# bootphon/abnet3

Hardware: AMD Instinct MI355X
Metric: frame-pairs/sec (Siamese train step: fwd both towers + coscos2 + bwd + Adadelta) (higher is better)
Workload: dtype f16x2; 1 GPU; C2: SiameseNetwork 40->500x2->100 sigmoid, coscos2(avg=False), Adadelta(0.1), 4096 frame pairs per GPU per step, 40-d N(0,1) frames; pairs_per_gpu=4096, global_pairs=4096, parallelism=dp1, graph_replay=False, dp_gradient_buckets=1

## Files before the change

### abnet3_amd/csrc/common.h

```cpp
#pragma once
#include <hip/hip_runtime.h>
#include <stdint.h>
#include <stdio.h>

#include "../../include/abnet3_hip.h"

namespace abn {

void set_error(const char* fmt, ...);

#define ABN_REQUIRE(cond, ...)                      \
    do {                                            \
        if (!(cond)) {                              \
            ::abn::set_error(__VA_ARGS__);          \
            return ABN_E_ARG;                       \
        }                                           \
    } while (0)

#define ABN_CHECK_LAUNCH(what)                                               \
    do {                                                                     \
        hipError_t e_ = hipGetLastError();                                   \
        if (e_ != hipSuccess) {                                              \
            ::abn::set_error("%s: %s", what, hipGetErrorString(e_));         \
            return ABN_E_LAUNCH;                                             \
        }                                                                    \
    } while (0)

struct Switches {
    bool planes;
    bool fused;
    int64_t fused_min_rows;
    bool bn_planes;
    bool bn_persist;
    bool wgrad_xcd;
    bool bf16x3_planes;
    bool bwd_pair;
    int gemm_tile;
    bool dtw_f40, dtw_pc;
    int wgrad_tile128;
    int dtw_wgs_per_cu;
    int wgrad_wgs_heavy, wgrad_wgs_light;
    int64_t wgrad_rows_per_slab;
    bool wide;
    int64_t wide_max_rows;
    int wide_max_groups;
    bool wgrad_step;
    bool dtw_dealt;
    int oneshot_wgs;
    int knn_split;
};
const Switches& switches();
void reload_switches();

// ... 23 lines not shown
```

### abnet3_amd/csrc/tower.hip

```cpp
#include <stdarg.h>
#include <stdlib.h>
#include <string.h>

#include <math.h>
#include <atomic>

#include "common.h"
#include "gemm_f32.h"
#include "opt_rule.h"
#include "tower_fused.h"
#include "tower_planes.h"
#include "tower_bn_persist.h"
#include "tower_wide.h"
#include "tower_wgrad_step.h"

namespace abn {

static thread_local char g_err[512] = "";
void set_error(const char* fmt, ...)
{
    va_list ap;
    va_start(ap, fmt);
    vsnprintf(g_err, sizeof(g_err), fmt, ap);
    va_end(ap);
// ... 10 lines not shown
    s.bn_persist = !off("ABN_BN_PERSIST");
    s.wgrad_xcd = !off("ABN_WGRAD_XCD");
    s.bf16x3_planes = !off("ABN_BF16X3_PLANES");
    s.bwd_pair = !off("ABN_BWD_PAIR");
    s.gemm_tile = getenv("ABN_GEMM_TILE") ? atoi(getenv("ABN_GEMM_TILE")) : -1;
    s.wgrad_rows_per_slab = getenv("ABN_WGRAD_ROWS_PER_SLAB") ? atoll(getenv("ABN_WGRAD_ROWS_PER_SLAB")) : -1;
    s.wide = !off("ABN_WIDE");
    s.wide_max_rows = getenv("ABN_WIDE_MAX_ROWS") ? atoll(getenv("ABN_WIDE_MAX_ROWS")) : -1;
    s.wide_max_groups = getenv("ABN_WIDE_MAXG") ? atoi(getenv("ABN_WIDE_MAXG")) : WD_MAXG;
    if (s.wide_max_groups < 1 || s.wide_max_groups > WD_MAXG) s.wide_max_groups = WD_MAXG;
    s.dtw_f40 = !off("ABN_DTW_F40");
    s.dtw_pc = !off("ABN_DTW_PC");
    s.wgrad_wgs_heavy = getenv("ABN_WGRAD_WGS_HEAVY") ? atoi(getenv("ABN_WGRAD_WGS_HEAVY")) : 128;
    s.wgrad_wgs_light = getenv("ABN_WGRAD_WGS_LIGHT") ? atoi(getenv("ABN_WGRAD_WGS_LIGHT")) : 128;
    s.wgrad_tile128 = getenv("ABN_WGRAD_TILE128") ? atoi(getenv("ABN_WGRAD_TILE128")) : -1;
    s.dtw_wgs_per_cu = getenv("ABN_DTW_WGS") ? atoi(getenv("ABN_DTW_WGS")) : 6;
    if (s.dtw_wgs_per_cu < 1 || s.dtw_wgs_per_cu > 9) s.dtw_wgs_per_cu = 6;
    s.wgrad_step = !off("ABN_WGRAD_STEP");
    s.dtw_dealt = !off("ABN_DTW_SCHED");
    s.oneshot_wgs = getenv("ABN_ONESHOT_WGS") ? atoi(getenv("ABN_ONESHOT_WGS")) : 32;
    if (s.oneshot_wgs < 1 || s.oneshot_wgs > 256) s.oneshot_wgs = 32;
    s.knn_split = getenv("ABN_KNN_SPLIT") ? atoi(getenv("ABN_KNN_SPLIT")) : 0;
    if (s.knn_split < 0) s.knn_split = 0;
    return s;
}
static Switches g_switches = read_switches();
const Switches& switches() { return g_switches; }
void reload_switches() { g_switches = read_switches(); }

template <int BM, int BN, bool A_KC, bool B_KC, int EPI, bool VEC, int BF16>
// ... 751 lines not shown
{
    bool all3 = np == 2 && w.n_layers > 0;
    for (int i = 0; i < w.n_layers; ++i) all3 = all3 && w.L[i].shape == 3;
    return all3;
}
constexpr size_t WGRAD128_LDS = (size_t)4 * 8 * 2048 + 128;
static void launch_wgrad(int np, const WgradP& w, int n_wg, hipStream_t st)
{
#ifndef WG128_GENERAL
    if (wgrad_all128(np, w)) {
        static bool attr_set[16] = {};
        int dev = 0;
        (void)hipGetDevice(&dev);
        dev = (dev >= 0 && dev < 16) ? dev : 0;
        if (!attr_set[dev]) {
            (void)hipFuncSetAttribute(reinterpret_cast<const void*>(wgrad_planes128_kernel), hipFuncAttributeMaxDynamicSharedMemorySize, (int)WGRAD128_LDS);
            attr_set[dev] = true;
        }
        hipLaunchKernelGGL(wgrad_planes128_kernel, dim3((unsigned)n_wg), dim3(PL_NT), WGRAD128_LDS, st, w);
        return;
    }
#endif
    PL_LAUNCH(np, wgrad_planes_kernel, dim3((unsigned)n_wg), dim3(PL_NT), wgrad_all128(np, w) ? WGRAD128_LDS : wgrad_lds_of(np), st, w);
}
static inline int gemm_prec(int precision) { return precision > 2 ? 2 : precision; }
static inline bool bn_sync_on(const abn_tower_desc* t) { return t->bn_sync_fn != nullptr && t->bn_sync_world >= 1; }
static inline int64_t bn_wgs_per_call(int64_t rows, int64_t n_calls) { return (rows / n_calls + PL_ROWS - 1) / PL_ROWS; }
static inline int64_t bn_vrows(int64_t rows, int64_t n_calls) { return n_calls * bn_wgs_per_call(rows, n_calls) * PL_ROWS; }
static bool planes_dims_ok(const abn_tower_desc* t)
{
    if (t->precision < 1) return false;
    for (int l = 0; l <= t->n_layers; ++l)
        if (t->dims[l] < 4 || t->dims[l] > PL_MAXW || t->dims[l] % 4 != 0) return false;
    return true;
// ... 176 lines not shown
    const int64_t n = in_dim + 1;
    const int64_t tm128 = (out_dim + 127) / 128, tm64 = (out_dim + 63) / 64;
    const int64_t tn128 = (n + 127) / 128, tn64 = (n + 63) / 64;
    const int64_t est = out_dim > 64 ? tm128 * tn64 : (n > 64 ? tm64 * tn128 : tm64 * tn64);
    int64_t s = (512 + est - 1) / est;
    const int64_t by_rows = rows / 128 < 1 ? 1 : rows / 128;
    if (s > by_rows) s = by_rows;
    if (s > MAX_SPLITS) s = MAX_SPLITS;
    return (int)(s < 1 ? 1 : s);
}

static inline bool wgrad_tile128(int64_t rows, bool np2)
{
    const int mode = switches().wgrad_tile128;
    return np2 && mode != 0 && (mode > 0 || (rows + 63) / 64 * 64 >= 2048);
}
static int planes_split_count(int64_t rows, int64_t out_dim, int64_t in_dim, bool np2 = false)
{
    int shape, bn, bk;
    const int nblk = pl_blocks(out_dim), kblk = pl_blocks(in_dim + 1);
    wgrad_shape(nblk, kblk, &shape, &bn, &bk, wgrad_tile128(rows, np2));
    const int64_t tiles = (int64_t)((nblk + bn - 1) / bn) * ((kblk + bk - 1) / bk);
    int64_t s = (128 + tiles - 1) / tiles;
    if (shape == 3) { const int64_t want = tiles >= 16 ? switches().wgrad_wgs_heavy : switches().wgrad_wgs_light; s = (want + tiles - 1) / tiles; }
    const int64_t r64 = (rows + 63) / 64 * 64;
    const int64_t per = switches().wgrad_rows_per_slab > 0 ? switches().wgrad_rows_per_slab : 128;
    const int64_t by_rows = r64 / per < 1 ? 1 : r64 / per;
    const int64_t cap = shape == 0 ? MAX_SPLITS : 2 * MAX_SPLITS;
    if (s > by_rows) s = by_rows;
    if (s > cap) s = cap;
// ... 335 lines not shown
    }
    b.a_top = ws + L.a[nl - 1];
    b.dx = dx;
    b.drop_seed = reinterpret_cast<const unsigned long long*>(t->drop_seed);
    b.drop_p = t->drop_p;
    const PackLayout PL = make_pack_layout(t);
    const char* const image = t->wpack ? reinterpret_cast<const char*>(t->wpack) : reinterpret_cast<const char*>(ws + L.wpack);
    for (int l = 0; l <= nl; ++l) b.dims[l] = (int)t->dims[l];
    for (int l = 0; l < nl; ++l) {
        b.act[l] = (l == nl - 1) ? t->last_act : t->act;
        b.tp[l] = reinterpret_cast<const char*>(ws + L.tp[l]);
        b.mask[l] = t->drop_mask[l];
        b.wpt[l] = image + PL.wpt[l];
        b.dzp[l] = reinterpret_cast<char*>(scratch + B.dzp[l]);
        b.amax_dz[l] = B.amax_dz[l] >= 0 ? scratch + B.amax_dz[l] : nullptr;
    }
    b.wbase = image; b.wbytes = PL.bytes;
    int l_first, l_end;
    { const int rc = wgrad_range(t, &l_first, &l_end); if (rc != ABN_OK) return rc; }
    if (t->wgrad_part == 2) part = PLANES_BWD_WGRAD;
    int n_wg = 0;
    const WgradP w = make_wgrad(t, rows, L, B, ws, scratch, &n_wg, l_first, l_end);
    static bool bw_attr_set[16] = {};
    int dev = 0;
    (void)hipGetDevice(&dev);
    dev = (dev >= 0 && dev < 16) ? dev : 0;
    if (!bw_attr_set[dev]) {
        PL_LDS_ATTR(tower_dgrad_planes_kernel, pl_lds_bytes);
        PL_LDS_ATTR(wgrad_planes_kernel, wgrad_lds_of);
        bw_attr_set[dev] = true;
    }
    const dim3 cgrid((unsigned)((rows + PL_ROWS - 1) / PL_ROWS));
    const bool do_dgrad = part != PLANES_BWD_WGRAD, do_wgrad = part != PLANES_BWD_DGRAD;
    if (do_dgrad) PL_LAUNCH(np, tower_dgrad_planes_kernel, cgrid, dim3(PL_NT), pl_lds_bytes(np), st, b);
    if (do_wgrad && n_wg > 0) launch_wgrad(np, w, n_wg, st);
    ABN_CHECK_LAUNCH("tower_backward (planes)");
    if (t->defer_reduce) return ABN_OK;
// ... 420 lines not shown
        const void* kernels[3][3] = {
            {reinterpret_cast<const void*>(tower_fwd_planes_kernel<1, PL_TRAIN>), reinterpret_cast<const void*>(tower_fwd_planes_kernel<1, PL_INFER>),
             reinterpret_cast<const void*>(tower_fwd_planes_kernel<1, PL_INFER_BN>)},
            {reinterpret_cast<const void*>(tower_fwd_planes_kernel<2, PL_TRAIN>), reinterpret_cast<const void*>(tower_fwd_planes_kernel<2, PL_INFER>),
             reinterpret_cast<const void*>(tower_fwd_planes_kernel<2, PL_INFER_BN>)},
            {reinterpret_cast<const void*>(tower_fwd_planes_kernel<3, PL_TRAIN>), reinterpret_cast<const void*>(tower_fwd_planes_kernel<3, PL_INFER>),
             reinterpret_cast<const void*>(tower_fwd_planes_kernel<3, PL_INFER_BN>)}};
        if (!pl_attr_set[dev]) {
            for (int a = 0; a < 3; ++a)
                for (int m = 0; m < 3; ++m)
                    if (kernels[a][m])
                        (void)hipFuncSetAttribute(kernels[a][m], hipFuncAttributeMaxDynamicSharedMemorySize,
                                                  (int)(m == PL_INFER_BN ? pl_lds_bytes_bn(a + 1) : pl_lds_bytes_stag(a + 1)));
            pl_attr_set[dev] = true;
        }
        void* kargs[] = {&f};
        (void)hipLaunchKernel(kernels[np - 1][mode], fgrid, dim3(PL_NT), kargs, lds, st);
        ABN_CHECK_LAUNCH("tower_fwd_planes");
        return ABN_OK;
    }
    if (fusable) {
        FusedFwdP f = {};
        f.n_layers = t->n_layers;
        f.rows = (int)rows;
        f.rows_call = (int)rpc;
        f.bf16 = gemm_prec(t->precision);
        f.x1 = x1; f.x2 = x2;
        f.x_copy = x2 ? ws + L.x : nullptr;
        for (int l = 0; l <= t->n_layers; ++l) f.dims[l] = (int)t->dims[l];
        for (int l = 0; l < t->n_layers; ++l) {
// ... 497 lines not shown
```

### abnet3_amd/csrc/tower_planes.h

```cpp
#pragma once
#include <type_traits>

#include "gemm_f32.h"

namespace abn {

typedef int v4i __attribute__((ext_vector_type(4)));

constexpr int PL_ROWS = 32;
constexpr int PL_WAVES = 8;
constexpr int PL_NT = 64 * PL_WAVES;
constexpr int PL_MAXW = 512;
constexpr int PL_MAXSTEPS = PL_MAXW / 16;
#ifdef PL_DEPTH_OVERRIDE
constexpr int PL_DEPTH = PL_DEPTH_OVERRIDE;
#else
constexpr int PL_DEPTH = 4;
#endif
constexpr int PL_PART_BYTES = 4 * 16 * 64 * 4;
constexpr int PL_SC_BYTES = PL_WAVES * 64 * 4 + PL_WAVES * 32 * 4;
constexpr int PL_AMAX = 32;

__host__ __device__ inline int pl_steps(int64_t contraction) { return ((int)((contraction + 15) / 16) + PL_DEPTH - 1) / PL_DEPTH * PL_DEPTH; }
__host__ __device__ inline int pl_blocks(int64_t features) { return (int)((features + 31) / 32); }
// ... 128 lines not shown
    for (int s = 0; s < 2; ++s) {
        if constexpr (NP == 2) {
            f16x8 o;
#pragma unroll
            for (int j = 0; j < 8; ++j) o[j] = (_Float16)((16 * s + 8 * (j >> 2) + 4 * h + (j & 3)) == c ? 1.0f : 0.0f);
            idf[s] = __builtin_bit_cast(bf16x8, o);
        } else {
#pragma unroll
            for (int j = 0; j < 8; ++j) idf[s][j] = (__bf16)((16 * s + 8 * (j >> 2) + 4 * h + (j & 3)) == c ? 1.0f : 0.0f);
        }
    }
}

template <int NP>
__device__ __forceinline__ void emit_planes(char* dst, const Frag<NP> f[2], const bf16x8 idf[2], int lane, int ones_c, int rows_left,
                                            const float* __restrict__ inv_tab = nullptr)
{
    const int c = lane & 31, h = lane >> 5;
    f32x16 t;
#pragma unroll
    for (int pl = 0; pl < NP; ++pl) {
        f32x16 u;
#pragma unroll
        for (int q = 0; q < 16; ++q) u[q] = 0.0f;
        u = pl_mfma<NP>(f[0].p[pl], idf[0], u);
        u = pl_mfma<NP>(f[1].p[pl], idf[1], u);
        if (pl == 0) t = u;
        else t += u;
    }
    if constexpr (NP == 2) {
#pragma unroll
        for (int g = 0; g < 4; ++g) {
            const f32x4 iv = *reinterpret_cast<const f32x4*>(inv_tab + 8 * g + 4 * h);
#pragma unroll
            for (int e = 0; e < 4; ++e) t[4 * g + e] *= iv[e];
        }
    }
    if (c == ones_c) {
#pragma unroll
        for (int q = 0; q < 16; ++q) t[q] = (q & 3) + 8 * (q >> 2) + 4 * h < rows_left ? 1.0f : 0.0f;
    }
#pragma unroll
    for (int s = 0; s < 2; ++s) {
        if constexpr (NP >= 2) {
            char* o = dst + s * 2048 + lane * 16;
            *reinterpret_cast<f32x4*>(o) = f32x4{t[8 * s], t[8 * s + 1], t[8 * s + 2], t[8 * s + 3]};
            *reinterpret_cast<f32x4*>(o + 1024) = f32x4{t[8 * s + 4], t[8 * s + 5], t[8 * s + 6], t[8 * s + 7]};
        } else {
            bf16x8 o;
#pragma unroll
            for (int j = 0; j < 8; ++j) o[j] = (__bf16)t[8 * s + j];
            *reinterpret_cast<bf16x8*>(dst + s * 1024 + lane * 16) = o;
        }
    }
}

template <int NP>
__device__ __forceinline__ int tgather_row_offset(int r)
{
    const int sp = r >> 4, jh = (r >> 3) & 1, jl = r & 3, hp = (r >> 2) & 1;
    if constexpr (NP >= 2) return sp * 2048 + jh * 1024 + hp * 32 * 16 + jl * 4;
    else return sp * 1024 + hp * 32 * 16 + (4 * jh + jl) * 2;
}
template <int NP>
__device__ __forceinline__ float tgather(const char* tile_pair, int row_off, int c)
{
    if constexpr (NP >= 2) return *reinterpret_cast<const float*>(tile_pair + row_off + c * 16);
    else return (float)*reinterpret_cast<const __bf16*>(tile_pair + row_off + c * 16);
}

template <int N> __device__ __forceinline__ void wait_vmcnt() { asm volatile("s_waitcnt vmcnt(%0)" :: "n"(N) : "memory"); }

struct PackJob {
    const float* W;
    int N, K;
    int transposed;
    int nblk, nsteps;
    int tile0;
    int blk0;
    int64_t dst;
};
struct PackTable {
    int n_jobs, n_tiles, n_blocks;
// ... 267 lines not shown
    int rows_call;
    int dims[ABN_MAX_LAYERS + 1];
    int act[ABN_MAX_LAYERS];
    const float* x1;
    const float* x2;
    float* x_copy;
    const char* wp[ABN_MAX_LAYERS];
    const char* wbase;
    int64_t wbytes;
    const float* b[ABN_MAX_LAYERS];
    const float* mask[ABN_MAX_LAYERS];
    float* out[ABN_MAX_LAYERS];
    char* tp[ABN_MAX_LAYERS];
    int64_t tp_steps;
    float* amax[ABN_MAX_LAYERS];
    const unsigned long long* drop_seed;
    float drop_p;
    const float* bn_rm[ABN_MAX_LAYERS];
    const float* bn_rv[ABN_MAX_LAYERS];
    const float* bn_w[ABN_MAX_LAYERS];
    const float* bn_b[ABN_MAX_LAYERS];
    float bn_eps;
    float* bn_part;
#ifdef ABN_STAMPS
    unsigned long long* stamps;
#endif
};

enum { PL_TRAIN = 0, PL_INFER = 1, PL_INFER_BN = 2, PL_BN_TRAIN = 3 };

// ... 334 lines not shown
        if (rescale) park_max();
    } else if (ws.active && ws.khalf == 1) {
#pragma unroll
        for (int q = 0; q < 16; ++q) part[((wave & 3) * 16 + q) * 64 + lane] = acc[0][q];
    }
    PSTAMPF(4 + 5 * l);
    __syncthreads();
    PSTAMPF(5 + 5 * l);
    if constexpr (STAGC) { if (stag_on) st.in_halves = false; }
    if (KS == 2 && ws.active && ws.khalf == 0) {
#pragma unroll
        for (int q = 0; q < 16; ++q) acc[0][q] += part[(wave * 16 + q) * 64 + lane];
        finish();
    }
    float osc = 1.0f;
    if (rescale) {
        if (KS == 2) { park_max(); __syncthreads(); }
        float oinv;
        const float m = row_scales(sc, wave, lane, osc, oinv);
        ainv = oinv;
        if (!INFER && p.tp[l + 1] && wave == 0) store_amax_rows(p.amax[l + 1] + (int64_t)blockIdx.x * PL_AMAX, m, 1.0f, lane);
    }
    const float* const inv_tab = sc + PL_WAVES * 64 + wave * 32;
    float* __restrict__ out = p.out[l];
    char* const tp = !INFER && !BNT && l + 1 < p.n_layers ? p.tp[l + 1] : nullptr;
    if (BNT && ws.active && ws.khalf == 0) {
        float* const pw = p.bn_part + (int64_t)blockIdx.x * (3 * PL_MAXW);
#pragma unroll
        for (int j = 0; j < BPW; ++j) {
            if (blk0 + j >= nblk) continue;
#pragma unroll
            for (int g = 0; g < 4; ++g) {
                f32x4 sd, sq, cc;
#pragma unroll
                for (int e = 0; e < 4; ++e) {
                    const float zv = acc[j][4 * g + e];
// ... 24 lines not shown
                Frag<NP> f[2];
#pragma unroll
                for (int t2 = 0; t2 < 2; ++t2) {
                    const f32x4 v0 = {acc[j][8 * t2], acc[j][8 * t2 + 1], acc[j][8 * t2 + 2], acc[j][8 * t2 + 3]};
                    const f32x4 v1 = {acc[j][8 * t2 + 4], acc[j][8 * t2 + 5], acc[j][8 * t2 + 6], acc[j][8 * t2 + 7]};
                    if (!BNT && (NP != 2 || rescale)) {
                        f[t2] = make_frag<NP>(v0, v1, osc);
                        store_frag<NP>(img + (int64_t)(2 * blk + t2) * (NP * 1024) + lane * 16, f[t2]);
                    }
                    const int n = 32 * blk + 16 * t2 + 4 * h;
                    if (out && row_ok && n < N) *reinterpret_cast<f32x4*>(out + (int64_t)gr * N + n) = v0;
                    if (out && row_ok && n + 8 < N) *reinterpret_cast<f32x4*>(out + (int64_t)gr * N + n + 8) = v1;
                }
                if (tp)
                    emit_planes<NP>(tp + ((int64_t)blk * p.tp_steps + 2 * blockIdx.x) * tile_bytes<NP>(), f, idf, lane,
                                    blk == N / 32 ? N % 32 : -1, rows_lim - row0, inv_tab);
            }
        }
    }
    if (tp && N % 32 == 0 && wave == PL_WAVES - 1) {
        Frag<NP> z[2] = {};
        emit_planes<NP>(tp + ((int64_t)nblk * p.tp_steps + 2 * blockIdx.x) * tile_bytes<NP>(), z, idf, lane, 0, rows_lim - row0, inv_tab);
    }
    PSTAMPF(6 + 5 * l);
    if (!BNT && l + 1 < p.n_layers) {
        const int next_steps = pl_steps(N);
        const bf16x8 z = {};
        for (int s = 2 * nblk + wave; s < next_steps; s += PL_WAVES)
#pragma unroll
            for (int pl = 0; pl < NP; ++pl) *reinterpret_cast<bf16x8*>(img + ((int64_t)s * NP + pl) * 1024 + lane * 16) = z;
    }
    __syncthreads();
}

template <int NP, bool INFER>
__device__ __forceinline__ void planes_input_stage(const PlanesFwdP& p, char* __restrict__ img, float* __restrict__ part,
                                                   const bf16x8* idf, int wave, int lane, int row0, float& ainv, int row_end = -1)
{
    const int rows_lim = row_end >= 0 ? row_end : p.rows;
    const int r = lane & 31, h = lane >> 5;
    const int D0 = p.dims[0];
    const int steps0 = pl_steps(D0), blocks0 = steps0 / 2;
    const int gr = row0 + r;
    const float* src = nullptr;
    if (gr < rows_lim) src = (p.x2 && gr >= p.rows_call) ? p.x2 + (int64_t)(gr - p.rows_call) * D0 : p.x1 + (int64_t)gr * D0;
    float* const sc = part + PL_PART_BYTES / 4;
    const float* const inv_tab = sc + PL_WAVES * 64 + wave * 32;
    if constexpr (NP == 2) {
        f32x4 v[2][2][2];
        float m = 0.0f;
#pragma unroll
        for (int u = 0; u < 2; ++u) {
            const int kb = wave + PL_WAVES * u;
#pragma unroll
            for (int t2 = 0; t2 < 2; ++t2) {
                const int c0 = 16 * (2 * kb + t2) + 4 * h, c1 = c0 + 8;
                v[u][t2][0] = v[u][t2][1] = f32x4{0.f, 0.f, 0.f, 0.f};
                if (src && kb < blocks0 && c0 < D0) {
                    v[u][t2][0] = *reinterpret_cast<const f32x4*>(src + c0);
                    if (p.x_copy) *reinterpret_cast<f32x4*>(p.x_copy + (int64_t)gr * D0 + c0) = v[u][t2][0];
                }
                if (src && kb < blocks0 && c1 < D0) {
                    v[u][t2][1] = *reinterpret_cast<const f32x4*>(src + c1);
                    if (p.x_copy) *reinterpret_cast<f32x4*>(p.x_copy + (int64_t)gr * D0 + c1) = v[u][t2][1];
                }
                m = fmaxf(m, absmax8(v[u][t2][0], v[u][t2][1]));
            }
        }
        sc[wave * 64 + lane] = m;
        __syncthreads();
        float osc;
        m = row_scales(sc, wave, lane, osc, ainv);
        if (!INFER && p.tp[0] && wave == 0) store_amax_rows(p.amax[0] + (int64_t)blockIdx.x * PL_AMAX, m, 1.0f, lane);
#pragma unroll
        for (int u = 0; u < 2; ++u) {
            const int kb = wave + PL_WAVES * u;
            if (kb < blocks0) {
                Frag<NP> f[2];
#pragma unroll
                for (int t2 = 0; t2 < 2; ++t2) {
                    f[t2] = make_frag<NP>(v[u][t2][0], v[u][t2][1], osc);
                    store_frag<NP>(img + (int64_t)(2 * kb + t2) * (NP * 1024) + lane * 16, f[t2]);
                }
                if (!INFER && p.tp[0] && kb < pl_blocks(D0 + 1))
                    emit_planes<NP>(p.tp[0] + ((int64_t)kb * p.tp_steps + 2 * blockIdx.x) * tile_bytes<NP>(), f, idf, lane,
                                    kb == D0 / 32 ? D0 % 32 : -1, rows_lim - row0, inv_tab);
            }
        }
    } else {
        for (int kb = wave; kb < blocks0; kb += PL_WAVES) {
            Frag<NP> f[2];
#pragma unroll
            for (int t2 = 0; t2 < 2; ++t2) {
                const int s = 2 * kb + t2;
                f32x4 v0 = {0.f, 0.f, 0.f, 0.f}, v1 = v0;
                const int c0 = 16 * s + 4 * h, c1 = c0 + 8;
                if (src && c0 < D0) {
                    v0 = *reinterpret_cast<const f32x4*>(src + c0);
                    if (p.x_copy) *reinterpret_cast<f32x4*>(p.x_copy + (int64_t)gr * D0 + c0) = v0;
                }
                if (src && c1 < D0) {
                    v1 = *reinterpret_cast<const f32x4*>(src + c1);
                    if (p.x_copy) *reinterpret_cast<f32x4*>(p.x_copy + (int64_t)gr * D0 + c1) = v1;
                }
                f[t2] = make_frag<NP>(v0, v1);
                store_frag<NP>(img + (int64_t)s * (NP * 1024) + lane * 16, f[t2]);
            }
            if (!INFER && p.tp[0] && kb < pl_blocks(D0 + 1))
                emit_planes<NP>(p.tp[0] + ((int64_t)kb * p.tp_steps + 2 * blockIdx.x) * tile_bytes<NP>(), f, idf, lane,
                                kb == D0 / 32 ? D0 % 32 : -1, rows_lim - row0);
        }
    }
    if (!INFER && p.tp[0] && pl_blocks(D0 + 1) > blocks0 && wave == PL_WAVES - 1) {
        Frag<NP> z[2] = {};
        emit_planes<NP>(p.tp[0] + ((int64_t)(D0 / 32) * p.tp_steps + 2 * blockIdx.x) * tile_bytes<NP>(), z, idf, lane, 0, rows_lim - row0, inv_tab);
    }
}

template <int NP, int MODE = PL_TRAIN>
__global__ __launch_bounds__(PL_NT) void tower_fwd_planes_kernel(PlanesFwdP p)
{
    constexpr bool INFER = MODE != PL_TRAIN;
    extern __shared__ __attribute__((aligned(16))) char pl_smem[];
    char* const img = pl_smem;
    float* const part = reinterpret_cast<float*>(pl_smem + PL_MAXSTEPS * NP * 1024);
    const int lane = threadIdx.x & 63;
    const int wave = __builtin_amdgcn_readfirstlane(threadIdx.x >> 6);
    const int row0 = blockIdx.x * PL_ROWS;
    bf16x8 idf[2];
    make_identity<NP>(idf, lane);
// ... 160 lines not shown
    int n_layers;
    int rows;
    int dims[ABN_MAX_LAYERS + 1];
    int act[ABN_MAX_LAYERS];
    const float* d_out;
    int d_out_is_dz;
    const float* a_top;
    const char* tp[ABN_MAX_LAYERS];
    float* dx;
    const float* mask[ABN_MAX_LAYERS];
    const char* wpt[ABN_MAX_LAYERS];
    const char* wbase;
    int64_t wbytes;
    char* dzp[ABN_MAX_LAYERS];
    float* amax_dz[ABN_MAX_LAYERS];
    int64_t tp_steps;
    const unsigned long long* drop_seed;
    float drop_p;
    int loss_kind;
    int y_dtype;
    const void* y;
    int B;
    double margin, scale;
    double* loss_partial;
    unsigned* loss_counter;
    float* loss_out;
    const int* n_valid;
    double* loss_accum;
#ifdef ABN_STAMPS
    unsigned long long* stamps;
// ... 46 lines not shown
            wv[j] = o + lane * 16;
            dnext[j] = ioff2 + blk2 * nsteps2 * (NP * 1024) - o;
        }
        if (ws.active) ring_kloop<NP, BPW>(acc, ring, wv, dnext, chain_next, img, ws.s_first, ws.my_steps, lane);
    }
    DSTAMP(4 + 4 * (p.n_layers - 1 - l));

    const float* __restrict__ mask = l >= 1 ? p.mask[l - 1] : nullptr;
    const DropGen drop = make_drop(l >= 1 && !mask ? p.drop_seed : nullptr, p.drop_p, l - 1);
    const bool masked = mask || drop.on;
    const int gr = row0 + r;
    const bool row_ok = gr < p.rows;
    const int grc = row_ok ? gr : p.rows - 1;
    f32x4 av[BPW][4], mv[BPW][4];
    if (ws.active && ws.khalf == 0 && l >= 1) {
        const int row_off = tgather_row_offset<NP>(r);
#pragma unroll
        for (int j = 0; j < BPW; ++j) {
            const int blk = blk0 + j < nblk ? blk0 + j : nblk - 1;
            const char* tile = p.tp[l] + ((int64_t)blk * p.tp_steps + 2 * blockIdx.x) * tile_bytes<NP>();
#pragma unroll
            for (int g = 0; g < 4; ++g) {
#pragma unroll
                for (int e = 0; e < 4; ++e) av[j][g][e] = tgather<NP>(tile, row_off, 8 * g + 4 * h + e);
                const int k = 32 * (blk0 + j) + 4 * h + 8 * g;
                if (mask) mv[j][g] = *reinterpret_cast<const f32x4*>(mask + (int64_t)grc * K + (k < K ? k : K - 4));
                else if (drop.on) mv[j][g] = drop4(drop, gr, k);
            }
        }
    }
    auto finish = [&]() {
        if constexpr (NP == 2) {
#pragma unroll
            for (int j = 0; j < BPW; ++j)
#pragma unroll
                for (int q = 0; q < 16; ++q) acc[j][q] *= cinv[j];
        }
        if (l == 0) return;
        with_act(p.act[l - 1], [&](auto tag) {
// ... 28 lines not shown
        if (ws.active) finish();
        if (rescale) park_max();
    } else if (ws.active && ws.khalf == 1) {
#pragma unroll
        for (int q = 0; q < 16; ++q) part[((wave & 3) * 16 + q) * 64 + lane] = acc[0][q];
    }
    DSTAMP(5 + 4 * (p.n_layers - 1 - l));
    __syncthreads();
    DSTAMP(6 + 4 * (p.n_layers - 1 - l));
    if (KS == 2 && ws.active && ws.khalf == 0) {
#pragma unroll
        for (int q = 0; q < 16; ++q) acc[0][q] += part[(wave * 16 + q) * 64 + lane];
        finish();
    }
    float osc = 1.0f;
    if (rescale) {
        if (KS == 2) { park_max(); __syncthreads(); }
        float oinv;
        const float m = row_scales(sc, wave, lane, osc, oinv);
        ainv = oinv;
        if (wave == 0) store_amax_rows(p.amax_dz[l - 1] + (int64_t)blockIdx.x * PL_AMAX, m, 0.0f, lane);
    }
    const float* const inv_tab = sc + PL_WAVES * 64 + wave * 32;
    if (ws.active && ws.khalf == 0) {
#pragma unroll
        for (int j = 0; j < BPW; ++j) {
            const int blk = blk0 + j;
            if (blk < nblk) {
                Frag<NP> f[2];
#pragma unroll
                for (int t2 = 0; t2 < 2; ++t2) {
                    const f32x4 v0 = {acc[j][8 * t2], acc[j][8 * t2 + 1], acc[j][8 * t2 + 2], acc[j][8 * t2 + 3]};
                    const f32x4 v1 = {acc[j][8 * t2 + 4], acc[j][8 * t2 + 5], acc[j][8 * t2 + 6], acc[j][8 * t2 + 7]};
                    if (l == 0) {
                        const int k = 32 * blk + 16 * t2 + 4 * h;
                        if (row_ok && k < K) *reinterpret_cast<f32x4*>(p.dx + (int64_t)gr * K + k) = v0;
                        if (row_ok && k + 8 < K) *reinterpret_cast<f32x4*>(p.dx + (int64_t)gr * K + k + 8) = v1;
                    } else {
                        f[t2] = make_frag<NP>(v0, v1, osc);
                        store_frag<NP>(img + (int64_t)(2 * blk + t2) * (NP * 1024) + lane * 16, f[t2]);
                    }
                }
                if (l >= 1) emit_planes<NP>(p.dzp[l - 1] + ((int64_t)blk * p.tp_steps + 2 * blockIdx.x) * tile_bytes<NP>(), f, idf, lane, -1, 0, inv_tab);
            }
        }
    }
    if (l - 1 >= 1 || (l == 1 && p.dx)) {
        const int next_steps = pl_steps(K);
        const bf16x8 z = {};
        for (int s = 2 * nblk + wave; s < next_steps; s += PL_WAVES)
#pragma unroll
            for (int pl = 0; pl < NP; ++pl) *reinterpret_cast<bf16x8*>(img + ((int64_t)s * NP + pl) * 1024 + lane * 16) = z;
    }
    __syncthreads();
    DSTAMP(7 + 4 * (p.n_layers - 1 - l));
}

template <int NP>
// ... 153 lines not shown
        float m = 0.0f;
#pragma unroll
        for (int u = 0; u < 2; ++u)
#pragma unroll
            for (int t2 = 0; t2 < 2; ++t2) {
                const int kb = wave + PL_WAVES * u;
                v[u][t2][0] = v[u][t2][1] = f32x4{0.f, 0.f, 0.f, 0.f};
                if (kb < blocks_t) top_step(2 * kb + t2, v[u][t2]);
                m = fmaxf(m, absmax8(v[u][t2][0], v[u][t2][1]));
            }
        sc[wave * 64 + lane] = m;
        __syncthreads();
        float osc;
        m = row_scales(sc, wave, lane, osc, ainv);
        if (wave == 0) store_amax_rows(p.amax_dz[top] + (int64_t)blockIdx.x * PL_AMAX, m, 0.0f, lane);
#pragma unroll
        for (int u = 0; u < 2; ++u) {
            const int kb = wave + PL_WAVES * u;
            if (kb < blocks_t) {
                Frag<NP> f[2];
#pragma unroll
                for (int t2 = 0; t2 < 2; ++t2) {
                    f[t2] = make_frag<NP>(v[u][t2][0], v[u][t2][1], osc);
                    store_frag<NP>(img + (int64_t)(2 * kb + t2) * (NP * 1024) + lane * 16, f[t2]);
                }
                if (kb < pl_blocks(NT))
                    emit_planes<NP>(p.dzp[top] + ((int64_t)kb * p.tp_steps + 2 * blockIdx.x) * tile_bytes<NP>(), f, idf, lane, -1, 0,
                                    sc + PL_WAVES * 64 + wave * 32);
            }
        }
    } else {
        for (int kb = wave; kb < blocks_t; kb += PL_WAVES) {
            Frag<NP> f[2];
#pragma unroll
            for (int t2 = 0; t2 < 2; ++t2) {
                f32x4 v[2];
                top_step(2 * kb + t2, v);
                f[t2] = make_frag<NP>(v[0], v[1]);
                store_frag<NP>(img + (int64_t)(2 * kb + t2) * (NP * 1024) + lane * 16, f[t2]);
            }
            if (kb < pl_blocks(NT))
                emit_planes<NP>(p.dzp[top] + ((int64_t)kb * p.tp_steps + 2 * blockIdx.x) * tile_bytes<NP>(), f, idf, lane, -1, 0);
        }
// ... 255 lines not shown
    int shape;
    int tiles_n, tiles_k;
    int splits;
    int first_wg;
    int64_t slab_off;
    const float* amax_dz;
    const float* amax_a;
};
struct WgradP {
    int n_layers;
    WgradLayer L[ABN_MAX_LAYERS];
    float* slabs;
    int64_t slab_stride;
    int64_t tp_steps;
    int xcd_groups;
#ifdef ABN_STAMPS
    unsigned long long* stamps;
#endif
};

__host__ __device__ inline int wgrad_group_count(int g0, int splits, int x, int* first)
{
    *first = g0 + ((x - g0) & 7);
    return *first < g0 + splits ? (g0 + splits - 1 - *first) / 8 + 1 : 0;
}
static inline int wgrad_slots(const WgradP& p, int x)
{
    int slots = 0, g0 = 0, first;
    for (int i = 0; i < p.n_layers; ++i) {
        slots += wgrad_group_count(g0, p.L[i].splits, x, &first) * p.L[i].tiles_n * p.L[i].tiles_k;
// ... 303 lines not shown
                tn = slot / p.L[li].tiles_k;
                return true;
            }
            slot -= cnt * G;
            g0 += p.L[li].splits;
        }
    }
    while (li + 1 < p.n_layers && (int)blockIdx.x >= p.L[li + 1].first_wg) ++li;
    int local = blockIdx.x - p.L[li].first_wg;
    tk = local % p.L[li].tiles_k; local /= p.L[li].tiles_k;
    tn = local % p.L[li].tiles_n; local /= p.L[li].tiles_n;
    split = local;
    return true;
}

#ifndef WG128_WAVES_PER_EU
#define WG128_WAVES_PER_EU 4
#endif
__global__ __launch_bounds__(PL_NT) __attribute__((amdgpu_waves_per_eu(WG128_WAVES_PER_EU, WG128_WAVES_PER_EU))) void wgrad_planes128_kernel(WgradP p)
{
    extern __shared__ __attribute__((aligned(16))) char wg_smem[];
    const int lane = threadIdx.x & 63;
    const int wave = __builtin_amdgcn_readfirstlane(threadIdx.x >> 6);
    int li, tk, tn, split;
    if (!wgrad_place(p, li, tn, tk, split)) return;
    const WgradLayer& L = p.L[li];
    const int s_begin = (int)(p.tp_steps * split / L.splits), s_end = (int)(p.tp_steps * (split + 1) / L.splits);
    wgrad_tile<2, 1, 2, 4, 2>(p, L, wg_smem, 4 * tn, 4 * tk, s_begin, s_end, split, wave, lane);
}

template <int NP>
__global__ __launch_bounds__(PL_NT) void wgrad_planes_kernel(WgradP p)
{
    extern __shared__ __attribute__((aligned(16))) char wg_smem[];
// ... 14 lines not shown
```

Measured before the change: 25.12 million frame-pairs/s.

## Emit pre-split f16 hi/lo plane images for wgrad and stream them via LDS DMA

When the 2-plane wgrad128 path applies, forward and backward now write activation and dz tiles as block-scaled f16 hi/lo planes instead of f32 rows. A new wgrad kernel loads these images straight into LDS with global_load_lds in a configurable multi-stage pipeline. It rescales each step's fragments by per-row-block amax factors and feeds them to f16 MFMA. This is meant to remove the in-kernel f32-to-plane conversion and shrink the staging traffic, at the cost of per-step scaling multiplies, an amax table pass, and some precision risk from rescaling in f16.

Result: slower. 23.78 million frame-pairs/s (-5.3%).

```diff
diff --git a/abnet3_amd/csrc/common.h b/abnet3_amd/csrc/common.h
--- a/abnet3_amd/csrc/common.h
+++ b/abnet3_amd/csrc/common.h
@@ -37,6 +37,7 @@
     bool bwd_pair;
     int gemm_tile;
     bool dtw_f40, dtw_pc;
+    int wgrad_image_stages;
     int wgrad_tile128;
     int dtw_wgs_per_cu;
     int wgrad_wgs_heavy, wgrad_wgs_light;
diff --git a/abnet3_amd/csrc/tower.hip b/abnet3_amd/csrc/tower.hip
--- a/abnet3_amd/csrc/tower.hip
+++ b/abnet3_amd/csrc/tower.hip
@@ -48,6 +48,8 @@
     s.wgrad_wgs_heavy = getenv("ABN_WGRAD_WGS_HEAVY") ? atoi(getenv("ABN_WGRAD_WGS_HEAVY")) : 128;
     s.wgrad_wgs_light = getenv("ABN_WGRAD_WGS_LIGHT") ? atoi(getenv("ABN_WGRAD_WGS_LIGHT")) : 128;
     s.wgrad_tile128 = getenv("ABN_WGRAD_TILE128") ? atoi(getenv("ABN_WGRAD_TILE128")) : -1;
+    s.wgrad_image_stages = getenv("ABN_WGRAD_IMAGE_STAGES") ? atoi(getenv("ABN_WGRAD_IMAGE_STAGES")) : 2;
+    if (s.wgrad_image_stages < 2 || s.wgrad_image_stages > 4) s.wgrad_image_stages = 2;
     s.dtw_wgs_per_cu = getenv("ABN_DTW_WGS") ? atoi(getenv("ABN_DTW_WGS")) : 6;
     if (s.dtw_wgs_per_cu < 1 || s.dtw_wgs_per_cu > 9) s.dtw_wgs_per_cu = 6;
     s.wgrad_step = !off("ABN_WGRAD_STEP");
@@ -829,10 +831,12 @@
         (void)hipGetDevice(&dev);
         dev = (dev >= 0 && dev < 16) ? dev : 0;
         if (!attr_set[dev]) {
-            (void)hipFuncSetAttribute(reinterpret_cast<const void*>(wgrad_planes128_kernel), hipFuncAttributeMaxDynamicSharedMemorySize, (int)WGRAD128_LDS);
+            (void)hipFuncSetAttribute(reinterpret_cast<const void*>(wgrad_planes128_f32_kernel), hipFuncAttributeMaxDynamicSharedMemorySize, (int)WGRAD128_LDS);
+            (void)hipFuncSetAttribute(reinterpret_cast<const void*>(wgrad_planes128_kernel), hipFuncAttributeMaxDynamicSharedMemorySize, (int)wgrad_image_lds_bytes(4));
             attr_set[dev] = true;
         }
-        hipLaunchKernelGGL(wgrad_planes128_kernel, dim3((unsigned)n_wg), dim3(PL_NT), WGRAD128_LDS, st, w);
+        if (w.plane_image) hipLaunchKernelGGL(wgrad_planes128_kernel, dim3((unsigned)n_wg), dim3(PL_NT), wgrad_image_lds_bytes(w.image_stages), st, w);
+        else hipLaunchKernelGGL(wgrad_planes128_f32_kernel, dim3((unsigned)n_wg), dim3(PL_NT), WGRAD128_LDS, st, w);
         return;
     }
 #endif
@@ -1039,6 +1043,10 @@
 {
     const int mode = switches().wgrad_tile128;
     return np2 && mode != 0 && (mode > 0 || (rows + 63) / 64 * 64 >= 2048);
+}
+static inline bool timage_planes(const abn_tower_desc* t, int64_t rows)
+{
+    return !PL_STAGGER && planes_of(t) == 2 && !t->batch_norm && wgrad_tile128(rows, true);
 }
 static int planes_split_count(int64_t rows, int64_t out_dim, int64_t in_dim, bool np2 = false)
 {
@@ -1404,13 +1412,17 @@
         b.wpt[l] = image + PL.wpt[l];
         b.dzp[l] = reinterpret_cast<char*>(scratch + B.dzp[l]);
         b.amax_dz[l] = B.amax_dz[l] >= 0 ? scratch + B.amax_dz[l] : nullptr;
-    }
+        b.amax_tp[l] = L.amax[l] >= 0 ? ws + L.amax[l] : nullptr;
+    }
+    b.tplanes = timage_planes(t, rows) ? 1 : 0;
     b.wbase = image; b.wbytes = PL.bytes;
     int l_first, l_end;
     { const int rc = wgrad_range(t, &l_first, &l_end); if (rc != ABN_OK) return rc; }
     if (t->wgrad_part == 2) part = PLANES_BWD_WGRAD;
     int n_wg = 0;
-    const WgradP w = make_wgrad(t, rows, L, B, ws, scratch, &n_wg, l_first, l_end);
+    WgradP w = make_wgrad(t, rows, L, B, ws, scratch, &n_wg, l_first, l_end);
+    w.plane_image = b.tplanes;
+    w.image_stages = switches().wgrad_image_stages;
     static bool bw_attr_set[16] = {};
     int dev = 0;
     (void)hipGetDevice(&dev);
@@ -1861,6 +1873,7 @@
                                                   (int)(m == PL_INFER_BN ? pl_lds_bytes_bn(a + 1) : pl_lds_bytes_stag(a + 1)));
             pl_attr_set[dev] = true;
         }
+        f.tplanes = mode == PL_TRAIN && timage_planes(t, rows) ? 1 : 0;
         void* kargs[] = {&f};
         (void)hipLaunchKernel(kernels[np - 1][mode], fgrid, dim3(PL_NT), kargs, lds, st);
         ABN_CHECK_LAUNCH("tower_fwd_planes");
diff --git a/abnet3_amd/csrc/tower_planes.h b/abnet3_amd/csrc/tower_planes.h
--- a/abnet3_amd/csrc/tower_planes.h
+++ b/abnet3_amd/csrc/tower_planes.h
@@ -166,7 +166,7 @@
 
 template <int NP>
 __device__ __forceinline__ void emit_planes(char* dst, const Frag<NP> f[2], const bf16x8 idf[2], int lane, int ones_c, int rows_left,
-                                            const float* __restrict__ inv_tab = nullptr)
+                                            const float* __restrict__ inv_tab = nullptr, float img_scale = 0.0f)
 {
     const int c = lane & 31, h = lane >> 5;
     f32x16 t;
@@ -191,6 +191,25 @@
     if (c == ones_c) {
 #pragma unroll
         for (int q = 0; q < 16; ++q) t[q] = (q & 3) + 8 * (q >> 2) + 4 * h < rows_left ? 1.0f : 0.0f;
+    }
+    if constexpr (NP == 2) {
+        if (img_scale != 0.0f) {
+            const float sc = c == ones_c ? 1.0f : img_scale;
+#pragma unroll
+            for (int s = 0; s < 2; ++s) {
+                u32x4p hi, lo;
+#pragma unroll
+                for (int i = 0; i < 4; ++i) {
+                    uint32_t hw, lw;
+                    split_f16x2_pair(sc, t[8 * s + 2 * i], t[8 * s + 2 * i + 1], hw, lw);
+                    hi[i] = hw; lo[i] = lw;
+                }
+                char* o = dst + s * 2048 + lane * 16;
+                *reinterpret_cast<u32x4p*>(o) = hi;
+                *reinterpret_cast<u32x4p*>(o + 1024) = lo;
+            }
+            return;
+        }
     }
 #pragma unroll
     for (int s = 0; s < 2; ++s) {
@@ -219,6 +238,24 @@
 {
     if constexpr (NP >= 2) return *reinterpret_cast<const float*>(tile_pair + row_off + c * 16);
     else return (float)*reinterpret_cast<const __bf16*>(tile_pair + row_off + c * 16);
+}
+
+__device__ __forceinline__ int tgather_row_offset_planes(int r)
+{
+    const int sp = r >> 4, jh = (r >> 3) & 1, jl = r & 3, hp = (r >> 2) & 1;
+    return sp * 2048 + hp * 32 * 16 + (4 * jh + jl) * 2;
+}
+__device__ __forceinline__ float tgather_planes(const char* tile_pair, int row_off, int c, float inv)
+{
+    const float hi = (float)*reinterpret_cast<const _Float16*>(tile_pair + row_off + c * 16);
+    const float lo = (float)*reinterpret_cast<const _Float16*>(tile_pair + row_off + c * 16 + 1024);
+    return (hi + lo) * inv;
+}
+__device__ __forceinline__ float block_scale(float m, float floor_)
+{
+    float s, inv;
+    scale_of(fmaxf(wave_max(m), floor_), s, inv);
+    return s;
 }
 
 template <int N> __device__ __forceinline__ void wait_vmcnt() { asm volatile("s_waitcnt vmcnt(%0)" :: "n"(N) : "memory"); }
@@ -516,6 +553,7 @@
     char* tp[ABN_MAX_LAYERS];
     int64_t tp_steps;
     float* amax[ABN_MAX_LAYERS];
+    int tplanes;
     const unsigned long long* drop_seed;
     float drop_p;
     const float* bn_rm[ABN_MAX_LAYERS];
@@ -880,12 +918,14 @@
         finish();
     }
     float osc = 1.0f;
+    float img_sc = 0.0f;
     if (rescale) {
         if (KS == 2) { park_max(); __syncthreads(); }
         float oinv;
         const float m = row_scales(sc, wave, lane, osc, oinv);
         ainv = oinv;
         if (!INFER && p.tp[l + 1] && wave == 0) store_amax_rows(p.amax[l + 1] + (int64_t)blockIdx.x * PL_AMAX, m, 1.0f, lane);
+        if (!INFER && p.tplanes) img_sc = block_scale(m, 1.0f);
     }
     const float* const inv_tab = sc + PL_WAVES * 64 + wave * 32;
     float* __restrict__ out = p.out[l];
@@ -940,13 +980,13 @@
                 }
                 if (tp)
                     emit_planes<NP>(tp + ((int64_t)blk * p.tp_steps + 2 * blockIdx.x) * tile_bytes<NP>(), f, idf, lane,
-                                    blk == N / 32 ? N % 32 : -1, rows_lim - row0, inv_tab);
+                                    blk == N / 32 ? N % 32 : -1, rows_lim - row0, inv_tab, img_sc);
             }
         }
     }
     if (tp && N % 32 == 0 && wave == PL_WAVES - 1) {
         Frag<NP> z[2] = {};
-        emit_planes<NP>(tp + ((int64_t)nblk * p.tp_steps + 2 * blockIdx.x) * tile_bytes<NP>(), z, idf, lane, 0, rows_lim - row0, inv_tab);
+        emit_planes<NP>(tp + ((int64_t)nblk * p.tp_steps + 2 * blockIdx.x) * tile_bytes<NP>(), z, idf, lane, 0, rows_lim - row0, inv_tab, img_sc);
     }
     PSTAMPF(6 + 5 * l);
     if (!BNT && l + 1 < p.n_layers) {
@@ -972,6 +1012,7 @@
     if (gr < rows_lim) src = (p.x2 && gr >= p.rows_call) ? p.x2 + (int64_t)(gr - p.rows_call) * D0 : p.x1 + (int64_t)gr * D0;
     float* const sc = part + PL_PART_BYTES / 4;
     const float* const inv_tab = sc + PL_WAVES * 64 + wave * 32;
+    float img_sc0 = 0.0f;
     if constexpr (NP == 2) {
         f32x4 v[2][2][2];
         float m = 0.0f;
@@ -998,6 +1039,7 @@
         float osc;
         m = row_scales(sc, wave, lane, osc, ainv);
         if (!INFER && p.tp[0] && wave == 0) store_amax_rows(p.amax[0] + (int64_t)blockIdx.x * PL_AMAX, m, 1.0f, lane);
+        if (!INFER && p.tplanes) img_sc0 = block_scale(m, 1.0f);
 #pragma unroll
         for (int u = 0; u < 2; ++u) {
             const int kb = wave + PL_WAVES * u;
@@ -1010,7 +1052,7 @@
                 }
                 if (!INFER && p.tp[0] && kb < pl_blocks(D0 + 1))
                     emit_planes<NP>(p.tp[0] + ((int64_t)kb * p.tp_steps + 2 * blockIdx.x) * tile_bytes<NP>(), f, idf, lane,
-                                    kb == D0 / 32 ? D0 % 32 : -1, rows_lim - row0, inv_tab);
+                                    kb == D0 / 32 ? D0 % 32 : -1, rows_lim - row0, inv_tab, img_sc0);
             }
         }
     } else {
@@ -1039,7 +1081,7 @@
     }
     if (!INFER && p.tp[0] && pl_blocks(D0 + 1) > blocks0 && wave == PL_WAVES - 1) {
         Frag<NP> z[2] = {};
-        emit_planes<NP>(p.tp[0] + ((int64_t)(D0 / 32) * p.tp_steps + 2 * blockIdx.x) * tile_bytes<NP>(), z, idf, lane, 0, rows_lim - row0, inv_tab);
+        emit_planes<NP>(p.tp[0] + ((int64_t)(D0 / 32) * p.tp_steps + 2 * blockIdx.x) * tile_bytes<NP>(), z, idf, lane, 0, rows_lim - row0, inv_tab, img_sc0);
     }
 }
 
@@ -1230,6 +1272,8 @@
     int64_t wbytes;
     char* dzp[ABN_MAX_LAYERS];
     float* amax_dz[ABN_MAX_LAYERS];
+    int tplanes;
+    const float* amax_tp[ABN_MAX_LAYERS];
     int64_t tp_steps;
     const unsigned long long* drop_seed;
     float drop_p;
@@ -1306,15 +1350,24 @@
     const int grc = row_ok ? gr : p.rows - 1;
     f32x4 av[BPW][4], mv[BPW][4];
     if (ws.active && ws.khalf == 0 && l >= 1) {
-        const int row_off = tgather_row_offset<NP>(r);
+        bool tplanes = false;
+        if constexpr (NP == 2) tplanes = p.tplanes != 0;
+        const int row_off = tplanes ? tgather_row_offset_planes(r) : tgather_row_offset<NP>(r);
+        float tinv = 1.0f;
+        if (tplanes) { float ts; scale_of(p.amax_tp[l][(int64_t)blockIdx.x * PL_AMAX], ts, tinv); }
 #pragma unroll
         for (int j = 0; j < BPW; ++j) {
             const int blk = blk0 + j < nblk ? blk0 + j : nblk - 1;
             const char* tile = p.tp[l] + ((int64_t)blk * p.tp_steps + 2 * blockIdx.x) * tile_bytes<NP>();
 #pragma unroll
             for (int g = 0; g < 4; ++g) {
-#pragma unroll
-                for (int e = 0; e < 4; ++e) av[j][g][e] = tgather<NP>(tile, row_off, 8 * g + 4 * h + e);
+                if (tplanes) {
+#pragma unroll
+                    for (int e = 0; e < 4; ++e) av[j][g][e] = tgather_planes(tile, row_off, 8 * g + 4 * h + e, tinv);
+                } else {
+#pragma unroll
+                    for (int e = 0; e < 4; ++e) av[j][g][e] = tgather<NP>(tile, row_off, 8 * g + 4 * h + e);
+                }
                 const int k = 32 * (blk0 + j) + 4 * h + 8 * g;
                 if (mask) mv[j][g] = *reinterpret_cast<const f32x4*>(mask + (int64_t)grc * K + (k < K ? k : K - 4));
                 else if (drop.on) mv[j][g] = drop4(drop, gr, k);
@@ -1373,12 +1426,14 @@
         finish();
     }
     float osc = 1.0f;
+    float img_sc = 0.0f;
     if (rescale) {
         if (KS == 2) { park_max(); __syncthreads(); }
         float oinv;
         const float m = row_scales(sc, wave, lane, osc, oinv);
         ainv = oinv;
         if (wave == 0) store_amax_rows(p.amax_dz[l - 1] + (int64_t)blockIdx.x * PL_AMAX, m, 0.0f, lane);
+        if (p.tplanes) img_sc = block_scale(m, 0.0f);
     }
     const float* const inv_tab = sc + PL_WAVES * 64 + wave * 32;
     if (ws.active && ws.khalf == 0) {
@@ -1400,7 +1455,7 @@
                         store_frag<NP>(img + (int64_t)(2 * blk + t2) * (NP * 1024) + lane * 16, f[t2]);
                     }
                 }
-                if (l >= 1) emit_planes<NP>(p.dzp[l - 1] + ((int64_t)blk * p.tp_steps + 2 * blockIdx.x) * tile_bytes<NP>(), f, idf, lane, -1, 0, inv_tab);
+                if (l >= 1) emit_planes<NP>(p.dzp[l - 1] + ((int64_t)blk * p.tp_steps + 2 * blockIdx.x) * tile_bytes<NP>(), f, idf, lane, -1, 0, inv_tab, img_sc);
             }
         }
     }
@@ -1584,6 +1639,7 @@
         float osc;
         m = row_scales(sc, wave, lane, osc, ainv);
         if (wave == 0) store_amax_rows(p.amax_dz[top] + (int64_t)blockIdx.x * PL_AMAX, m, 0.0f, lane);
+        const float img_sc = p.tplanes ? block_scale(m, 0.0f) : 0.0f;
 #pragma unroll
         for (int u = 0; u < 2; ++u) {
             const int kb = wave + PL_WAVES * u;
@@ -1596,7 +1652,7 @@
                 }
                 if (kb < pl_blocks(NT))
                     emit_planes<NP>(p.dzp[top] + ((int64_t)kb * p.tp_steps + 2 * blockIdx.x) * tile_bytes<NP>(), f, idf, lane, -1, 0,
-                                    sc + PL_WAVES * 64 + wave * 32);
+                                    sc + PL_WAVES * 64 + wave * 32, img_sc);
             }
         }
     } else {
@@ -1882,6 +1938,8 @@
     int64_t slab_stride;
     int64_t tp_steps;
     int xcd_groups;
+    int plane_image;
+    int image_stages;
 #ifdef ABN_STAMPS
     unsigned long long* stamps;
 #endif
@@ -2215,10 +2273,163 @@
     return true;
 }
 
+constexpr int WGI_STAGE_BYTES = 8 * 2 * 2 * 1024;
+constexpr int WGI_CHUNK = 64;
+constexpr int WGI_TAB_BYTES = 128 + WGI_CHUNK * 8;
+static inline size_t wgrad_image_lds_bytes(int stages) { return (size_t)stages * WGI_STAGE_BYTES + WGI_TAB_BYTES; }
+
+template <int NS>
+__device__ __forceinline__ void wgrad_tile_image(const WgradP& p, const WgradLayer& L, char* __restrict__ smem, int nb0, int kb0,
+                                                 int s_begin, int s_end, int split, int wave, int lane)
+{
+    constexpr int WN = 4, TK = 2, BN = 4;
+    const int wn = wave % WN, wk = wave / WN;
+    const int n_steps = s_end - s_begin;
+    const int rb0 = s_begin >> 1, rb_end = (s_end + 1) >> 1, n_stages = rb_end - rb0;
+    const int rb_last = (int)(p.tp_steps >> 1) - 1;
+    const bool is_dz = wave < BN;
+    const int ob = is_dz ? nb0 + wave : kb0 + (wave - BN);
+    const int ob_max = is_dz ? L.nblk : L.kblk;
+    const char* const src = (is_dz ? L.dzp : L.ap) + (int64_t)(ob < ob_max ? ob : ob_max - 1) * p.tp_steps * 2048 + lane * 16;
+    auto dma = [&](int c) {
+        const int rb = rb0 + c < rb_last ? rb0 + c : rb_last;
+        char* const dst = smem + (c % NS) * WGI_STAGE_BYTES + wave * 4096;
+#pragma unroll
+        for (int d = 0; d < 4; ++d)
+            __builtin_amdgcn_global_load_lds((const __attribute__((address_space(1))) void*)(src + (int64_t)rb * 4096 + d * 1024),
+                                             (__attribute__((address_space(3))) void*)(dst + d * 1024), 16, 0, 0);
+    };
+    f32x16 acc[TK];
+#pragma unroll
+    for (int j = 0; j < TK; ++j)
+#pragma unroll
+        for (int q = 0; q < 16; ++q) acc[j][q] = 0.0f;
+    const bool live = nb0 + wn < L.nblk && kb0 + wk * TK < L.kblk;
+
+#pragma unroll
+    for (int c = 0; c < NS - 1; ++c) dma(c);
+
+    float* const red = reinterpret_cast<float*>(smem + NS * WGI_STAGE_BYTES);
+    float* const tab = red + 32;
+    float sd, sa, id, ia;
+    {
+        const int cnt = n_stages * PL_AMAX;
+        float md = 0.0f, ma = 0.0f;
+        for (int i = threadIdx.x; i < cnt; i += PL_NT) {
+            md = fmaxf(md, L.amax_dz[(int64_t)rb0 * PL_AMAX + i]);
+            ma = fmaxf(ma, L.amax_a[(int64_t)rb0 * PL_AMAX + i]);
+        }
+        md = wave_max(md); ma = wave_max(ma);
+        if (lane == 0) { red[wave] = md; red[8 + wave] = ma; }
+        __syncthreads();
+#pragma unroll
+        for (int w = 0; w < PL_WAVES; ++w) { md = fmaxf(md, red[w]); ma = fmaxf(ma, red[8 + w]); }
+        scale_of(md, sd, id);
+        scale_of(ma, sa, ia);
+    }
+    auto fill_tab = [&](int c0) {
+        __syncthreads();
+        if (threadIdx.x < WGI_CHUNK && c0 + (int)threadIdx.x < n_stages) {
+            const int64_t rb = rb0 + c0 + threadIdx.x;
+            float s_, bd, ba;
+            scale_of(L.amax_dz[rb * PL_AMAX], s_, bd);
+            scale_of(L.amax_a[rb * PL_AMAX], s_, ba);
+            tab[2 * threadIdx.x] = sd * bd;
+            tab[2 * threadIdx.x + 1] = sa * ba;
+        }
+        asm volatile("s_waitcnt vmcnt(0)" ::: "memory");
+        __syncthreads();
+    };
+    fill_tab(0);
+    const int ones_blk = L.K / 32 - kb0 - wk * TK;
+    const bool ones_lane = (lane & 31) == L.K % 32;
+
+    struct Frags { f16x8 a[2], b[TK][2]; };
+    auto read_frags = [&](Frags& f, int c, int step) {
+        const char* st = smem + (c % NS) * WGI_STAGE_BYTES + step * 2048 + lane * 16;
+#pragma unroll
+        for (int pl = 0; pl < 2; ++pl) {
+            f.a[pl] = *reinterpret_cast<const f16x8*>(st + wn * 4096 + pl * 1024);
+#pragma unroll
+            for (int j = 0; j < TK; ++j) f.b[j][pl] = *reinterpret_cast<const f16x8*>(st + (BN + wk * TK + j) * 4096 + pl * 1024);
+        }
+    };
+    auto scale_frags = [&](Frags& f, float fa, float fb) {
+        if (fa != 1.0f) {
+            const _Float16 m = (_Float16)fa;
+#pragma unroll
+            for (int pl = 0; pl < 2; ++pl) f.a[pl] *= m;
+        }
+        if (fb != 1.0f) {
+#pragma unroll
+            for (int j = 0; j < TK; ++j) {
+                const _Float16 m = (_Float16)(ones_lane && j == ones_blk ? 1.0f : fb);
+#pragma unroll
+                for (int pl = 0; pl < 2; ++pl) f.b[j][pl] *= m;
+            }
+        }
+    };
+    auto mfmas = [&](const Frags& f) {
+#pragma unroll
+        for (int u = 0; u < Products<2>::N; ++u)
+#pragma unroll
+            for (int j = 0; j < TK; ++j)
+                acc[j] = __builtin_amdgcn_mfma_f32_32x32x16_f16(f.a[Products<2>::A[u]], f.b[j][Products<2>::B[u]], acc[j], 0, 0, 0);
+    };
+    for (int c = 0; c < n_stages; ++c) {
+        if (c && c % WGI_CHUNK == 0) fill_tab(c);
+        wait_vmcnt<(NS - 2) * 4>();
+        __syncthreads();
+        dma(c + NS - 1);
+        const float rd = __int_as_float(__builtin_amdgcn_readfirstlane(__float_as_int(tab[2 * (c % WGI_CHUNK)])));
+        const float ra = __int_as_float(__builtin_amdgcn_readfirstlane(__float_as_int(tab[2 * (c % WGI_CHUNK) + 1])));
+        const int s0 = 2 * (rb0 + c);
+        const float fa0 = s0 >= s_begin && s0 < s_end ? rd : 0.0f, fa1 = s0 + 1 >= s_begin && s0 + 1 < s_end ? rd : 0.0f;
+        if (live) {
+            Frags f0, f1;
+            read_frags(f0, c, 0);
+            read_frags(f1, c, 1);
+            scale_frags(f0, fa0, ra);
+            mfmas(f0);
+            scale_frags(f1, fa1, ra);
+            mfmas(f1);
+        }
+    }
+    asm volatile("s_waitcnt vmcnt(0)" ::: "memory");
+
+    const float out_inv = id * ia, out_inv_ones = id;
+    float* const slab = p.slabs + (int64_t)split * p.slab_stride + L.slab_off;
+    const int h = lane >> 5;
+#pragma unroll
+    for (int j = 0; j < TK; ++j) {
+        const int k = 32 * (kb0 + wk * TK + j) + (lane & 31);
+        if (k <= L.K) {
+#pragma unroll
+            for (int q = 0; q < 16; ++q) {
+                const int n = 32 * (nb0 + wn) + (q & 3) + 8 * (q >> 2) + 4 * h;
+                if (n < L.N) slab[k < L.K ? (int64_t)n * L.K + k : (int64_t)L.N * L.K + n] = acc[j][q] * (k < L.K ? out_inv : out_inv_ones);
+            }
+        }
+    }
+}
+
 #ifndef WG128_WAVES_PER_EU
 #define WG128_WAVES_PER_EU 4
 #endif
 __global__ __launch_bounds__(PL_NT) __attribute__((amdgpu_waves_per_eu(WG128_WAVES_PER_EU, WG128_WAVES_PER_EU))) void wgrad_planes128_kernel(WgradP p)
+{
+    extern __shared__ __attribute__((aligned(16))) char wg_smem[];
+    const int lane = threadIdx.x & 63;
+    const int wave = __builtin_amdgcn_readfirstlane(threadIdx.x >> 6);
+    int li, tk, tn, split;
+    if (!wgrad_place(p, li, tn, tk, split)) return;
+    const WgradLayer& L = p.L[li];
+    const int s_begin = (int)(p.tp_steps * split / L.splits), s_end = (int)(p.tp_steps * (split + 1) / L.splits);
+    if (p.image_stages == 4) wgrad_tile_image<4>(p, L, wg_smem, 4 * tn, 4 * tk, s_begin, s_end, split, wave, lane);
+    else if (p.image_stages == 3) wgrad_tile_image<3>(p, L, wg_smem, 4 * tn, 4 * tk, s_begin, s_end, split, wave, lane);
+    else wgrad_tile_image<2>(p, L, wg_smem, 4 * tn, 4 * tk, s_begin, s_end, split, wave, lane);
+}
+__global__ __launch_bounds__(PL_NT) __attribute__((amdgpu_waves_per_eu(WG128_WAVES_PER_EU, WG128_WAVES_PER_EU))) void wgrad_planes128_f32_kernel(WgradP p)
 {
     extern __shared__ __attribute__((aligned(16))) char wg_smem[];
     const int lane = threadIdx.x & 63;
```
